# QuEraComputing/tsim

Measured on AMD Instinct MI355X. Metric: detector shots/sec, 35-qubit distillation circuit, 1/2/4/8 MI355X, higher is better.
Workload: dtype int32

## Files before the change

include/tsim_hip.h:

```cpp
#ifndef TSIM_HIP_H
#define TSIM_HIP_H

#include <stdint.h>

#ifdef __cplusplus
extern "C" {
#endif

#define TSIM_OK 0
#define TSIM_EINVAL (-22)
#define TSIM_ENOMEM (-12)
#define TSIM_EHIP (-5)
#define TSIM_ENOTSUP (-95)
#define TSIM_ESTATE (-1)

#define TSIM_MAX_PARAMS 2048

typedef struct tsim_program tsim_program;

typedef struct tsim_level_desc {
  int32_t num_graphs;
  int32_t n_params;
  int32_t ta, tb, tc, td;
  const uint8_t *a_phases;
// ... 303 lines not shown
int tsim_profile_read_stages(tsim_program *p, double stage_ms[3]);
int tsim_profile_read_steps(tsim_program *p, int64_t *steps, int32_t reset);


int tsim_program_info(const tsim_program *p, int32_t *n_components, int32_t *num_outputs,
                      int64_t *image_bytes, int64_t *total_graphs, int64_t *total_rows);

int tsim_program_stats(const tsim_program *p, int64_t out[8]);

#define TSIM_PATH_COUNT 24
int tsim_program_path_counts(tsim_program *p, int64_t out[TSIM_PATH_COUNT], int32_t reset);

const char *tsim_last_error(void);
const char *tsim_version(void);
const char *tsim_tune_keys(void);

#ifdef __cplusplus
}
#endif
#endif
```

tsim_amd/_lib.py:

```python

from __future__ import annotations

import ctypes as C
import os
from pathlib import Path

import numpy as np

_HERE = Path(__file__).resolve().parent
LIB_PATH = _HERE / "libtsim_hip.so"


class HipBackendError(RuntimeError):
    """The HIP extension is missing, failed to load, or a call into it failed."""


class LevelDesc(C.Structure):

    _fields_ = [
        ("num_graphs", C.c_int32),
        ("n_params", C.c_int32),
        ("ta", C.c_int32),
        ("tb", C.c_int32),
        ("tc", C.c_int32),
# ... 178 lines not shown
    "tsim_program_path_counts": (C.c_int, [_P, C.POINTER(_I64), C.c_int32]),
    "tsim_key_split": (None, [_U32, _U32, C.POINTER(_U32)]),
    "tsim_sample_batch_device_begin_split": (C.c_int, [_P, _I32, _P, _I64, _I32, C.POINTER(_U32), _I64, _P, _P, _P, _U32]),
    "tsim_sample_steps_device": (C.c_int, [_P, _I32, C.POINTER(_P), _I64, _I32, C.POINTER(_U32), _I64, C.POINTER(_P), C.POINTER(_P), _U32]),
    "tsim_sample_steps_noise_device": (C.c_int, [_P, _P, _I32, C.POINTER(_P), _I64, _I32, C.POINTER(_U32), C.POINTER(_U32), _I64, C.POINTER(_P),
                                                 C.POINTER(_P), _U32]),
    "tsim_profile_read_steps": (C.c_int, [_P, C.POINTER(_I64), _I32]),
    "tsim_memcpy_d2h_async": (C.c_int, [_P, _P, _P, _I64, _P]),
    "tsim_memcpy_h2d_async": (C.c_int, [_P, _P, _P, _I64, _P]),
    "tsim_stream_synchronize": (C.c_int, [_P, _P]),
    "tsim_aux_stream": (C.c_int, [_P, _I32, C.POINTER(_P)]),
    "tsim_pipeline_next_slot": (C.c_int, [_P, C.POINTER(_I32)]),
    "tsim_last_error": (C.c_char_p, []),
    "tsim_version": (C.c_char_p, []),
    "tsim_tune_keys": (C.c_char_p, []),
}

_lib = None


def load(build: bool = True) -> C.CDLL:
    global _lib
    if _lib is not None:
        return _lib
    path = Path(os.environ.get("TSIM_AMD_LIB", LIB_PATH))
    if path == LIB_PATH:
        from . import build as _build

        if _build.needs_build():
            if path.exists() and os.environ.get("TSIM_AMD_ALLOW_STALE") == "1":
# ... 59 lines not shown
```

tsim_amd/csrc/tsim_internal.hip.h:

```cpp
#pragma once
#include "tsim_host.hip.h"
#include "tsim_kernels.hip.h"
#include "tsim_kernel4.hip.h"
#ifndef TSIM_HARD_NW
#define TSIM_HARD_NW 8
#endif
#include "tsim_lw.hip.h"

#include <algorithm>
#include <array>
#include <cstdarg>
#include <cstdio>
#include <cstdlib>
#include <cmath>
#include <atomic>
#include <mutex>
#include <chrono>
#include <cstring>
#include <functional>
#include <new>
#include <string>
#include <thread>
#include <unordered_set>
#include <vector>

#define TSIMK_H_MAX_CTX 8
constexpr int kListRows = 40;
constexpr int kMinLists = 4;
constexpr int kHardLdsKb = 128;
constexpr int kV4Block = 256;
constexpr int kWideGlobGraphs = 48;

void tsim_parallel_for_impl(size_t n, int max_threads, const std::function<void(size_t)> &fn);
template <class F>
inline void tsim_parallel_for(size_t n, int max_threads, F &&fn) {
  tsim_parallel_for_impl(n, max_threads, std::function<void(size_t)>(std::forward<F>(fn)));
}

namespace tsimhost {

struct FastGraph {
// ... 176 lines not shown
  int lw_direct_left = 0;
  struct Knobs {
    bool adaptive = true;
    bool fused_steps = true;
    int deep_tables = 0;
    bool defer = true;
    int defer_group = 4;
    bool lw_fast = true;
    bool wide_fused = true;
    bool hard_wave = true;
    int hard_wave_rows = 1024;
    long long hard_inline_rows = 1ll << 40;
    bool hard_comp_par = true;
    unsigned long long deep_after = 0;
    int fused_lanes = 0;
    int fused_max = 8;
    bool wide_tables = true;
    bool hard_overflow = true;
    bool shallow = true;
    bool noise_fused = true;
    int trie = 1;
    int gen = 1;
    int x4 = 32;
    bool x3 = true;
    int wide_depth = 4;
    int wide_passes = 8;
    bool wide_compact = true;
  } knobs;
  bool h_attr_set = false;
  bool hm_attr_set = false;
  unsigned gen_attr_set = 0;
// ... 101 lines not shown
```

tsim_amd/csrc/tsim_kernel4.hip.h:

```cpp
#pragma once
#include "tsim_kernels.hip.h"

namespace tsimk {

enum { L4_G = 0, L4_NTILES, L4_TABLES, L4_RECS, L4_NCH, L4_FLAGS, L4_FRAME, L4_STAB, L4_WORDS = 8 };
enum {
  G4_M0 = 0, G4_M1, G4_M3, G4_PM, G4_N1, G4_DBITS , G4_TBL, G4_FLAGS, G4_TBL2,
  G4_CFIELD = 9 ,
  G4_APRE = 11, G4_APIM = 12, G4_WORDS = 16
};
#define TSIMK_G4FLAG_D_COMBINED 1u
#define TSIMK_G4FLAG_D_SEPARATE 2u
enum { C4_LEVELS = 8, C4_WORDS = 16 };

#ifndef TSIMK_V4_WAVES
#define TSIMK_V4_WAVES 1
#endif

struct Sample4Args {
  SampleArgs s;
  int comp4_off;
  int has_check;
  uint32_t *feedback;
};
// ... 335 lines not shown
    }
    if (check_block && threadIdx.x == 0 && active && A.norm_dev) A.norm_dev[ci] = maxdev;
  }

  if (active && !check_block) {
    if (A.out) {
      uint64_t *orow = A.out + row * A.WO;
      for (int w = 0; w < A.WO; ++w)
        orow[w] = (uint64_t)lds_o[(2 * w) * nthr] | ((uint64_t)lds_o[(2 * w + 1) * nthr] << 32);
    }
    store_compact_row(A, row, lds_o, nthr);
  }
}

#ifndef TSIMK_H_MAX_CTX
#define TSIMK_H_MAX_CTX 8
#endif
struct Over4Multi {
  int n_ctx, comp4_off;
  uint32_t slot_begin;
  int masked;
  SampleArgs ctx[TSIMK_H_MAX_CTX];
};

template <int GT, int NCH>
__device__ __forceinline__ void over4_rows(const SampleArgs *ctx, int n_ctx, int comp4_off, uint32_t slot_begin, bool masked,
                                           uint32_t worker, uint32_t n_workers) {
  const uint32_t nthr = blockDim.x;
  __shared__ uint32_t s_cnt[TSIMK_H_MAX_CTX * 64];
  {
    bool any = false;
// ... 41 lines not shown
```

tsim_amd/csrc/tsim_kernel4h.hip.h:

```cpp
#pragma once
#include "tsim_kernel4.hip.h"

namespace tsimk {

#define TSIMK_H_MAX_GROUP_TILES 12

template <int GT, int NCH, int NW>
struct Hard4 {
  static constexpr int kMaxPerWave = (TSIMK_H_MAX_GROUP_TILES * GT + NW - 1) / NW;
  static constexpr int kTileBytes = NCH * Tile4<GT>::kChunkBytes;
  static constexpr int kExchWords = NW * 8 * 64;
};

__device__ __forceinline__ void h4_index(cptr gr, uint32_t U, uint32_t V, uint32_t O1, uint32_t O2, uint32_t &idx,
                                         uint32_t &dbits, uint32_t &r) {
  const uint32_t gflags = gr[G4_FLAGS];
  const bool z = (O1 & gr[G4_M0]) != 0;
  const uint32_t m1 = (uint32_t)__builtin_popcount(O1 & gr[G4_M1]);
  const uint32_t m3 = (uint32_t)__builtin_popcount(O1 & gr[G4_M3]);
  idx = m3 - m1 + gr[G4_N1];
  const uint32_t dsh = gr[G4_DBITS];
  dbits = O2 & ((1u << dsh) - 1u);
  if (gflags & TSIMK_G4FLAG_D_COMBINED) idx = (idx << dsh) | dbits;
  idx = z ? 0u : idx + 1u;
// ... 285 lines not shown
    }
    store_compact_row(A, row, lds_o, 64);
  }
  if (check_block || loop_stride <= 0 || !A.row_index) return;
  __syncthreads();
  }
}

template <int GT, int NCH, int NW>
__global__ void __launch_bounds__(NW * 64) __attribute__((amdgpu_waves_per_eu(3, 8))) k_sample4h(Sample4Args A4, int group_tiles, int loop_stride,
                                                        uint32_t *feedback) {
  sample4h_rows<GT, NCH, NW>(A4.s, A4.comp4_off, A4.has_check != 0, group_tiles, loop_stride, feedback, blockIdx.x,
                             gridDim.x);
}

#define TSIMK_H_MAX_CTX 8
struct Hard4Multi {
  int n_ctx, blocks_per_ctx, group_tiles, loop_stride;
  int comp4_off, check_mask;
  uint32_t *feedback;
  uint32_t main_blocks, over_from;
  SampleArgs ctx[TSIMK_H_MAX_CTX];
};

template <int GT, int NCH, int NW>
__global__ void __launch_bounds__(NW * 64) __attribute__((amdgpu_waves_per_eu(3, 8))) k_sample4h_multi(Hard4Multi M) {
  if (blockIdx.x >= M.main_blocks) {
    over4_rows<GT, NCH>(M.ctx, M.n_ctx, M.comp4_off, M.over_from, false, blockIdx.x - M.main_blocks, gridDim.x - M.main_blocks);
    return;
  }
  const uint32_t c = blockIdx.x / (uint32_t)M.blocks_per_ctx;
// ... 10 lines not shown
```

tsim_amd/csrc/tsim_kernel_hw.hip.h:

```cpp
#pragma once
#include "tsim_kernels.hip.h"
#include "tsim_kernel4.hip.h"

namespace tsimk {

#define TSIMK_HW_MAX_CTX 8
struct HwMulti {
  int n_ctx, waves_per_list, max_lists;
  int comp_par;
  int par_words;
  uint32_t slot_cap;
  uint32_t hw_blocks;
  int comp4_off;
  uint32_t *feedback;
  SampleArgs ctx[TSIMK_HW_MAX_CTX];
};

__device__ __forceinline__ int hw_sum_i32(int v) {
#pragma unroll
  for (int o = 32; o > 0; o >>= 1) v += __shfl_xor(v, o, 64);
  return v;
}
__device__ __forceinline__ uint32_t hw_or_u32(uint32_t v) {
#pragma unroll
// ... 419 lines not shown
```

tsim_amd/csrc/tsim_lw_fast.hip.h:

```cpp
#pragma once
#include "tsim_lw_multi.hip.h"

namespace tsimk {

enum { LWF_NRUNS = 0, LWF_FLIP0, LWF_FLIP1, LWF_RUNS ,
       LWF_RANK , LWF_LUT , LWF_NOUT, LWF_WORDS = 16 };
#define TSIMK_LWF_MAX_RUNS 32
#define TSIMK_LWF_MAX_NOUT 8

__device__ __forceinline__ uint32_t threefry_bits32_lo(uint32_t k0, uint32_t k1, uint32_t k0hi, uint32_t lo) {
  const uint32_t k2 = k0 ^ k1 ^ 0x1BD11BDAu;
  uint32_t x0, x1, t;
#define TF_RN(r) "v_alignbit_b32 %[x1], %[x1], %[x1], " #r "\n v_xor_b32 %[x1], %[x1], %[x0]\n"
#define TF_RA(r) "v_add_u32 %[x0], %[x0], %[x1]\n" TF_RN(r)
#define TF_INJ(kb, i, ka) "s_add_i32 %[t], %[" #kb "], " #i "\n v_add_u32 %[x1], %[t], %[x1]\n v_add3_u32 %[x0], %[x0], %[x1], %[" #ka "]\n"
  asm("v_add_u32 %[x1], %[k1], %[lo]\n v_add_u32 %[x0], %[k0hi], %[x1]\n"
      TF_RN(19) TF_RA(17) TF_RA(6) TF_RA(26)
      TF_INJ(k2, 1, k1) TF_RN(15) TF_RA(3) TF_RA(16) TF_RA(8)
      TF_INJ(k0, 2, k2) TF_RN(19) TF_RA(17) TF_RA(6) TF_RA(26)
      TF_INJ(k1, 3, k0) TF_RN(15) TF_RA(3) TF_RA(16) TF_RA(8)
      TF_INJ(k2, 4, k1) TF_RN(19) TF_RA(17) TF_RA(6) TF_RA(26)
      "s_add_i32 %[t], %[k0], 5\n v_add_u32 %[x0], %[k2], %[x0]\n v_add_u32 %[x1], %[t], %[x1]\n v_xor_b32 %[x0], %[x0], %[x1]\n"
      : [x0] "=&v"(x0), [x1] "=&v"(x1), [t] "=&s"(t)
      : [lo] "v"(lo), [k0] "s"(k0), [k1] "s"(k1), [k2] "s"(k2), [k0hi] "s"(k0hi)
// ... 7 lines not shown
template <int WF32, int NOUT>
__global__ void __launch_bounds__(1024) __attribute__((amdgpu_num_sgpr(TSIMK_LW_SGPRS))) k_sample_lw_fast(LwMultiArgs M) {
  typedef const __attribute__((address_space(4))) uint8_t *cbytes;
  typedef const __attribute__((address_space(4))) LwStep *cstep;
  typedef uint32_t u32x2 __attribute__((ext_vector_type(2)));
  typedef uint32_t u32x4 __attribute__((ext_vector_type(4)));
  constexpr int NPOS = 32 * WF32;
  constexpr int RSTR = NPOS + 1;
  constexpr int L_RANK = 0;
  constexpr int L_LUT = (L_RANK + 8 * RSTR + 1) & ~1;
  constexpr int L_RUNS = L_LUT + (2 << NOUT);
  constexpr int L_BASES = L_RUNS + 4 * TSIMK_LWF_MAX_RUNS;
  constexpr int L_WORDS = L_BASES + 72;
  __shared__ uint32_t lds[L_WORDS];
  const int nthr = blockDim.x;
  cptr img = (cptr)(uintptr_t)M.img;
  cptr rec = img + M.lw_off;
  cptr fr = img + M.lwf_off;
  {
    const uint32_t *g = M.img;
    const uint32_t rank_off = fr[LWF_RANK], lut_off = fr[LWF_LUT], runs_off = fr[LWF_RUNS], n_runs = fr[LWF_NRUNS];
    for (int i = threadIdx.x; i < 8 * RSTR; i += nthr)
      lds[L_RANK + i] = (i % RSTR) < NPOS ? g[rank_off + (uint32_t)(i / RSTR) * 128u + (uint32_t)(i % RSTR)] : 0u;
    for (int i = threadIdx.x; i < (2 << NOUT); i += nthr) lds[L_LUT + i] = g[lut_off + i];
    for (int i = threadIdx.x; i < 4 * TSIMK_LWF_MAX_RUNS; i += nthr) lds[L_RUNS + i] = (uint32_t)i < 4u * n_runs ? g[runs_off + i] : 0u;
    if (threadIdx.x < 72) lds[L_BASES + threadIdx.x] = threadIdx.x < 8 ? g[M.lw_off + LW_BASES_INLINE + threadIdx.x] : 0u;
    __syncthreads();
  }
  const uint32_t n_runs = fr[LWF_NRUNS], flip0 = fr[LWF_FLIP0], flip1 = fr[LWF_FLIP1];
  uint32_t sel[4];
#pragma unroll
  for (int w = 0; w < 4; ++w) sel[w] = w < WF32 ? rec[LW_SEL_INLINE + w] : 0u;
  const uint32_t wmax = rec[LW_WMAX];
  const uint32_t tab_byte = rec[LW_TAB] * 4u;
  const uint32_t keybase = rec[LW_KEYBASE];
  const __amdgpu_buffer_rsrc_t r_tab = __builtin_amdgcn_make_buffer_rsrc((void *)M.tab, 0, M.tab_bytes, 0x00020000);
  cstep steps = (cstep)((cbytes)__builtin_amdgcn_kernarg_segment_ptr() + __builtin_offsetof(LwMultiArgs, step));
  const uint32_t so_lo = (uint32_t)M.shot_offset, so_hi = (uint32_t)((unsigned long long)M.shot_offset >> 32);

  const uint32_t bps = (uint32_t)M.blocks_per_step;
  const uint32_t total = bps * (uint32_t)M.n_steps;
  uint32_t vb = blockIdx.x;
  if (vb >= total) return;
  uint32_t step = vb / bps, rb = vb - step * bps;
  const uint32_t Bu = (uint32_t)M.B;
  uint32_t n[4] = {0u, 0u, 0u, 0u};
  auto load_f = [&](uint32_t st, uint32_t rbk) {
    const __amdgpu_buffer_rsrc_t r_f = __builtin_amdgcn_make_buffer_rsrc((void *)steps[st].f, 0, Bu * (uint32_t)(4 * WF32), 0x00020000);
    const uint32_t row = rbk * (uint32_t)nthr + threadIdx.x;
    const uint32_t off = row * (uint32_t)(4 * WF32);
    if (TSIMK_LWM_SKIP & 64) { n[0] ^= (row * 0x9E3779B9u) & (row * 0x85EBCA6Bu) & (row * 0xC2B2AE35u) & 0x11111111u; n[1] = 0; return; }
    if constexpr (WF32 == 2) {
      const u32x2 v = __builtin_amdgcn_raw_buffer_load_b64(r_f, off, 0, 0);
      n[0] = v.x; n[1] = v.y;
    } else {
      const u32x4 v = __builtin_amdgcn_raw_buffer_load_b128(r_f, off, 0, 0);
      n[0] = v.x; n[1] = v.y; n[2] = v.z; n[3] = v.w;
    }
  };
  load_f(step, rb);
  for (;;) {
    cstep S = steps + step;
    const uint32_t row = rb * (uint32_t)nthr + threadIdx.x;
    const bool active = row < Bu;
    uint32_t f[4] = {n[0], n[1], n[2], n[3]};
    uint32_t vb_n = vb + gridDim.x, step_n = step, rb_n = rb + gridDim.x;
    while (rb_n >= bps) { rb_n -= bps; ++step_n; }
    const bool more = vb_n < total;
    if (more) load_f(step_n, rb_n);
    if (rb == 0u && threadIdx.x <= TSIMK_LW_LISTS)
      S->ctl_next[32u * threadIdx.x] = (threadIdx.x == TSIMK_LW_LISTS) ? 0xFFFFFFFFu : 0u;
    uint32_t o0 = 0u, o1 = 0u;
    for (uint32_t r = 0; r < ((TSIMK_LWM_SKIP & 2) ? 0u : n_runs); ++r) {
      const u32x4 run = *reinterpret_cast<const u32x4 *>(&lds[L_RUNS + 4u * r]);
      const uint32_t sw = (uint32_t)__builtin_amdgcn_readfirstlane((int)run.x) >> 8;
// ... 140 lines not shown
```

tsim_amd/csrc/tsim_lw_multi.hip.h:

```cpp
#pragma once
#include "tsim_lw_pass.hip.h"

namespace tsimk {

#ifndef TSIMK_LWM_SKIP
#define TSIMK_LWM_SKIP 0
#endif

#define TSIMK_LWM_MAX_STEPS 16
#define TSIMK_LWM_KEYS 16

struct LwStep {
  const uint64_t *f;
  uint64_t *out;
  uint8_t *out_compact;
  uint32_t *hard_index;
  uint32_t *ctl;
  uint32_t *ctl_next;
  uint32_t keys[2 * TSIMK_LWM_KEYS];
};

struct LwMultiArgs {
  const uint32_t *img;
  const uint32_t *tab;
  long long B;
  long long shot_offset;
  int n_steps, blocks_per_step;
  int n_comp, lw_off, direct_rot, binom_off;
  int has_check, list_cap, n_lists, out_rb;
  int lwf_off;
  uint32_t tab_bytes;
  int partial;
  LwStep step[TSIMK_LWM_MAX_STEPS];
};

template <int WF32>
__device__ __forceinline__ void lwm_load_f(const uint64_t *f, long long row, bool active, uint32_t &f0, uint32_t &f1, uint32_t &f2,
                                           uint32_t &f3) {
  f0 = f1 = f2 = f3 = 0u;
  if (TSIMK_LWM_SKIP & 64) {
    f0 = ((uint32_t)row * 0x9E3779B9u) & ((uint32_t)row * 0x85EBCA6Bu) & ((uint32_t)row * 0xC2B2AE35u) & 0x11111111u;
    return;
  }
  if (active) {
    const uint64_t *frow = f + row * (WF32 / 2);
    const uint64_t v0 = frow[0];
    f0 = (uint32_t)v0;
// ... 134 lines not shown
```

tsim_amd/csrc/tsim_program.hip:

```cpp
#include "tsim_internal.hip.h"
#include <map>
#include "tsim_sample_internal.hip.h"
#include "tsim_lw_fastm.hip.h"
#include "tsim_kernel4w.hip.h"
#include "tsim_wide.hip.h"
#include "tsim_gen.hip.h"

using namespace tsimk;
using namespace tsimhost;

static thread_local char g_err[512] = "";

bool tsim_debug(const char *what) {
  const char *e = getenv("TSIM_AMD_DEBUG");
  return e && strstr(e, what) != nullptr;
}

int tsim_fail(int code, const char *fmt, ...) {
  va_list ap;
  va_start(ap, fmt);
  vsnprintf(g_err, sizeof g_err, fmt, ap);
  va_end(ap);
  return code;
}
// ... 228 lines not shown
extern "C" int tsim_program_finalize(tsim_program *p, int32_t device) {
  if (!p) return tsim_fail(TSIM_EINVAL, "program is NULL");
  if (p->finalized) return tsim_fail(TSIM_ESTATE, "program already finalized");
  {
    auto env_int = [](const char *name, int dflt) { const char *e = getenv(name); return e ? atoi(e) : dflt; };
    const std::string tune = getenv("TSIM_AMD_TUNE") ? std::string(",") + getenv("TSIM_AMD_TUNE") + "," : std::string();
    auto tune_ll = [&](const char *key, long long dflt) -> long long {
      const std::string k = std::string(",") + key + "=";
      const size_t at = tune.find(k);
      return at == std::string::npos ? dflt : atoll(tune.c_str() + at + k.size());
    };
    p->knobs.adaptive = env_int("TSIM_AMD_ADAPTIVE", 1) != 0;
    p->knobs.fused_steps = env_int("TSIM_AMD_FUSED_STEPS", 1) != 0;
    p->knobs.deep_tables = env_int("TSIM_AMD_DEEP_TABLES", 0);
    p->knobs.defer = tune_ll("defer_hard", 1) != 0;
    p->knobs.defer_group = (int)std::max(0ll, std::min((long long)TSIMK_H_MAX_CTX, tune_ll("defer_group", 0)));
    p->knobs.lw_fast = tune_ll("lw_fast", 1) != 0;
    p->knobs.wide_fused = tune_ll("wide_fused", 1) != 0;
    p->knobs.hard_wave = tune_ll("hard_wave", 1) != 0;
    p->knobs.hard_wave_rows = (int)std::max(0ll, tune_ll("hard_wave_rows", 1024));
    p->knobs.hard_inline_rows = std::max(0ll, tune_ll("hard_inline_rows", 1ll << 40));
    p->knobs.hard_comp_par = tune_ll("hard_comp_par", 1) != 0;
    p->knobs.deep_after = (unsigned long long)std::max(0ll, tune_ll("deep_after", 0));
    p->knobs.fused_lanes = (int)std::max(0ll, std::min(4ll, tune_ll("fused_lanes", 0)));
    p->knobs.fused_max = (int)std::max(1ll, std::min((long long)TSIMK_LWM_MAX_STEPS, tune_ll("fused_max", 8)));
    p->knobs.wide_tables = tune_ll("wide_tables", 1) != 0;
    p->knobs.wide_compact = tune_ll("wide_compact", 1) != 0;
    p->knobs.x3 = tune_ll("x3", 1) != 0;
    p->knobs.x4 = (int)std::max(0ll, tune_ll("x4", 32));
    p->knobs.wide_depth = (int)std::max(0ll, std::min(4ll, tune_ll("wide_depth", 4)));
    p->knobs.wide_passes = (int)std::max(1ll, std::min(16ll, tune_ll("wide_passes", 8)));
    p->knobs.gen = (int)std::max(0ll, std::min(2ll, tune_ll("gen", 1)));
    p->knobs.trie = (int)std::max(0ll, std::min(2ll, tune_ll("trie", 1)));
    p->knobs.noise_fused = tune_ll("noise_fused", 1) != 0;
    p->knobs.shallow = tune_ll("shallow", 1) != 0;
    p->knobs.hard_overflow = tune_ll("hard_overflow", 1) != 0;
  }

  const bool fin_dbg = tsim_debug("finalize");
  auto fin_t0 = std::chrono::steady_clock::now();
// ... 975 lines not shown
        }
      } else {
        p->lw_wmax.clear();
      }
    }
  }
  if (p->lw) {
    while (img.size() % 32) img.push_back(0u);
    p->lw_shadow_off = (int)img.size();
    img.resize(img.size() + p->comps.size() * LW_WORDS, 0u);
  }
  img.resize(img.size() + 256, 0u);
  if (img.size() >= (1ull << 30)) return tsim_fail(TSIM_ENOTSUP, "program image too large");

  if (p->knobs.defer_group <= 0)
    p->knobs.defer_group = p->stats[5] > (4ll << 20) ? TSIMK_H_MAX_CTX : 4;

  fin_mark("pattern-table plan, first-pass records");
  int ndev = 0;
  HIP_TRY(hipGetDeviceCount(&ndev));
  if (device < 0 || device >= ndev) return tsim_fail(TSIM_EINVAL, "device %d out of range (%d visible)", device, ndev);
  p->device = device;
  HIP_TRY(hipSetDevice(device));
  {
    int cu = 0;
    if (hipDeviceGetAttribute(&cu, hipDeviceAttributeMultiprocessorCount, device) == hipSuccess && cu > 0) p->n_cu = cu;
  }
  if (int r = tsim_stream_acquire(device, p->stream_idx, &p->stream)) return r;
  HIP_TRY(hipMalloc((void **)&p->d_img, img.size() * 4));
  HIP_TRY(hipMemcpy(p->d_img, img.data(), img.size() * 4, hipMemcpyHostToDevice));
  HIP_TRY(hipMalloc((void **)&p->d_dev, std::max<size_t>(1, p->comps.size()) * 4));
// ... 285 lines not shown
```

tsim_amd/csrc/tsim_sample.hip:

```cpp
#include "tsim_internal.hip.h"

#include <chrono>
#include "tsim_kernel4h.hip.h"
#include "tsim_filter.hip.h"
#include "tsim_lw_pass.hip.h"
#include "tsim_lw_multi.hip.h"
#include "tsim_lw_fast.hip.h"
#include "tsim_kernel4w.hip.h"
#include "tsim_kernel_hw.hip.h"
#include "tsim_direct.hip.h"
#include "tsim_lw_fastm.hip.h"
#include "tsim_sample_internal.hip.h"
#include "tsim_noise_fused.hip.h"

using namespace tsimk;
using namespace tsimhost;

thread_local TsimNoiseRequest *g_noise_req = nullptr;
HostMarks *g_marks = nullptr;


int prof_event(tsim_program *p, hipStream_t s, int tag) {
  if (p->ev_used == p->ev_pool.size()) {
    hipEvent_t e;
// ... 172 lines not shown
static int slots_now_ready(tsim_program *p) {
  p->slots_ready = true;
  return 0;
}
static thread_local const LaunchPlan *g_carry_plan = nullptr;

void hard_geometry(tsim_program *p, int WF, int WO) {
  constexpr int NW = TSIM_HARD_NW;
  const size_t tile_b = (size_t)p->v4_max_nch * 16 * p->v4_gt * 16;
  const size_t fixed_b = (size_t)(2 * WF + 2 * WO) * 64 * 4 + (size_t)NW * 8 * 64 * 4;
  const size_t budget = (size_t)kHardLdsKb * 1024;
  p->h_group_tiles = fixed_b + tile_b <= budget ? (int)std::min<size_t>(TSIMK_H_MAX_GROUP_TILES, (budget - fixed_b) / tile_b) : 0;
  p->h_lds = fixed_b + (size_t)std::max(1, p->h_group_tiles) * tile_b;
}

static bool hw_eligible(tsim_program *p, const SampleArgs &a, int n_ctx) {
  int wmax = 1;
  for (int w : p->comp_w) wmax = std::max(wmax, w);
  const uint32_t fb_rows = p->h_feedback ? p->h_feedback[0] : 0u;
  return p->fast && p->knobs.hard_wave && wmax <= 4 && a.WF <= 32 && a.WO <= 2 && p->hw_max_rows < 60000 &&
         (unsigned long long)fb_rows * (unsigned)n_ctx <= (unsigned long long)p->knobs.hard_wave_rows;
}
static int launch_over(tsim_program *p, const SampleArgs *ctx, int n_ctx, uint32_t slot_begin, bool masked, hipStream_t hs, bool fill_chip = false) {
  Over4Multi M{};
  M.n_ctx = n_ctx;
  M.comp4_off = p->comp4_off;
  M.slot_begin = slot_begin;
  M.masked = masked ? 1 : 0;
  for (int i = 0; i < n_ctx; ++i) {
    M.ctx[i] = ctx[i];
// ... 1 lines not shown
    M.ctx[i].row_slot_begin = 0;
    M.ctx[i].row_slot_end = 0;
  }
  const int blk = 256;
  const size_t tile_bytes = std::max((size_t)p->v4_max_nch * 16, (size_t)p->v4_max_sent) * p->v4_gt * 16;
  const size_t lds4 = (size_t)(2 * ctx[0].WF + 2 * ctx[0].WO) * blk * 4 + 2 * tile_bytes;
  if (lds4 > (p->v4_max_nch == 32 ? 160 : 64) * 1024) return tsim_fail(TSIM_ENOTSUP, "v4 kernel needs %zu B of LDS", lds4);
  const unsigned grid = (unsigned)p->n_cu * (fill_chip ? (unsigned)std::max<size_t>(1, std::min<size_t>(2048 / blk, (160 * 1024) / (lds4 + 256))) : 1u);
  ++p->path_count[TP_OVER];
  switch (p->v4_max_nch) {
#define TSIM_LO(N) case N: hipLaunchKernelGGL((k_sample4_over<4, N>), dim3(grid), dim3(blk), lds4, hs, M); break;
    TSIM_LO(2) TSIM_LO(4) TSIM_LO(6) TSIM_LO(8) TSIM_LO(10) TSIM_LO(12) TSIM_LO(14) TSIM_LO(20)
#undef TSIM_LO
    case 32: {
      auto kfn = k_sample4_over<4, 32>;
      if (!(p->x4_attr_set & 1u)) { HIP_TRY(hipFuncSetAttribute((const void *)kfn, hipFuncAttributeMaxDynamicSharedMemorySize, 160 * 1024 - 4096)); p->x4_attr_set |= 1u; }
      hipLaunchKernelGGL(kfn, dim3(grid), dim3(blk), lds4, hs, M);
    } break;
    default: hipLaunchKernelGGL((k_sample4_over<4, 16>), dim3(grid), dim3(blk), lds4, hs, M); break;
  }
  HIP_TRY(hipGetLastError());
  return 0;
}
static bool over_available(const tsim_program *p) { return p->v4 && p->knobs.hard_overflow; }

static int launch_hw(tsim_program *p, const SampleArgs *ctx, int n_ctx, int max_lists, hipStream_t hs, bool partial, bool with_feedback = true) {
  int wmax = 1;
  for (int w : p->comp_w) wmax = std::max(wmax, w);
  const uint32_t fb_max = p->h_feedback ? p->h_feedback[1] : 192u;
  HwMulti H{};
  H.n_ctx = n_ctx;
// ... 21 lines not shown
  }
  const int nch = workers ? p->v4_max_nch : 0;
  ++p->path_count[TP_HW];
#define TSIM_LHW(WV, N) case N: hipLaunchKernelGGL((k_sample_hw<WV, N>), dim3(grid), dim3(256), ldsw, hs, H); break;
  if (wmax == 1) switch (nch) {
    TSIM_LHW(1, 0) TSIM_LHW(1, 2) TSIM_LHW(1, 4) TSIM_LHW(1, 6) TSIM_LHW(1, 8) TSIM_LHW(1, 10) TSIM_LHW(1, 12) TSIM_LHW(1, 14) TSIM_LHW(1, 16)
    default: return tsim_fail(TSIM_ESTATE, "bad chunk count %d", nch);
  } else if (wmax > 4) {
    if (nch != 0 || wmax > 8) return tsim_fail(TSIM_ESTATE, "block-per-row kernel: %d parameter words, %d chunks", wmax, nch);
    hipLaunchKernelGGL((k_sample_hw<8, 0>), dim3(grid), dim3(256), ldsw, hs, H);
  } else if (wmax > 2) {
    switch (nch) {
      TSIM_LHW(4, 0) TSIM_LHW(4, 20)
      case 32: {
        auto kfn = k_sample_hw<4, 32>;
        if (!(p->x4_attr_set & 2u)) { HIP_TRY(hipFuncSetAttribute((const void *)kfn, hipFuncAttributeMaxDynamicSharedMemorySize, 160 * 1024 - 4096)); p->x4_attr_set |= 2u; }
        hipLaunchKernelGGL(kfn, dim3(grid), dim3(256), ldsw, hs, H);
      } break;
      default: return tsim_fail(TSIM_ESTATE, "hard-row workers need chunk tables (%d chunks)", nch);
    }
  } else switch (nch) {
    TSIM_LHW(2, 0) TSIM_LHW(2, 2) TSIM_LHW(2, 4) TSIM_LHW(2, 6) TSIM_LHW(2, 8) TSIM_LHW(2, 10) TSIM_LHW(2, 12) TSIM_LHW(2, 14) TSIM_LHW(2, 16)
    default: return tsim_fail(TSIM_ESTATE, "bad chunk count %d", nch);
  }
#undef TSIM_LHW
  HIP_TRY(hipGetLastError());
  return 0;
}

int flush_batch(tsim_program *p) {
  if (p->deferred.empty()) {
// ... 56 lines not shown
  if (cap4h && !over_apart) {
    const size_t tile_bytes = std::max((size_t)p->v4_max_nch * 16, (size_t)p->v4_max_sent) * p->v4_gt * 16;
    lds_m = std::max(lds_m, (size_t)(2 * M.ctx[0].WF + 2 * M.ctx[0].WO) * (NW * 64) * 4 + 2 * tile_bytes);
    grid += (unsigned)p->n_cu * (many ? 2u : 1u);
  }
  if (over_apart) {
    for (hipEvent_t &e : p->over_ev)
      if (!e) HIP_TRY(hipEventCreateWithFlags(&e, hipEventDisableTiming));
    HIP_TRY(hipEventRecord(p->over_ev[0], hs));
  }
  switch (p->v4_max_nch) {
#define TSIM_LHM(N)                                                                                          \
  case N: {                                                                                                  \
    auto kfn = k_sample4h_multi<4, N, NW>;                                                                   \
    if (!p->hm_attr_set)                             \
      HIP_TRY(hipFuncSetAttribute((const void *)kfn, hipFuncAttributeMaxDynamicSharedMemorySize, 156 * 1024)); \
    ++p->path_count[TP_SAMPLE4H_MULTI];                                                                      \
    hipLaunchKernelGGL(kfn, dim3(grid), dim3(NW * 64), lds_m, hs, M);                                        \
  } break;
    TSIM_LHM(2) TSIM_LHM(4) TSIM_LHM(6) TSIM_LHM(8) TSIM_LHM(10) TSIM_LHM(12) TSIM_LHM(14) TSIM_LHM(16) TSIM_LHM(20) TSIM_LHM(32)
#undef TSIM_LHM
    default: return tsim_fail(TSIM_ESTATE, "bad chunk count %d", p->v4_max_nch);
  }
  HIP_TRY(hipGetLastError());
  p->hm_attr_set = true;
  if (over_apart) {
    hipStream_t os = p->slots[4].side != hs ? p->slots[4].side : p->slots[3].side;
    HIP_TRY(hipStreamWaitEvent(os, p->over_ev[0], 0));
    if (int r = launch_over(p, M.ctx, M.n_ctx, cap4h, false, os, true)) return r;
    HIP_TRY(hipEventRecord(p->over_ev[1], os));
    HIP_TRY(hipStreamWaitEvent(hs, p->over_ev[1], 0));
// ... 295 lines not shown
      M.tab = p->d_lw_tab;
      M.B = B;
      M.shot_offset = shot_offset;
      M.n_steps = 1;
      M.blocks_per_step = (int)blocks;
      M.n_comp = (int)p->comps.size();
      M.lw_off = p->lw_off;
      M.direct_rot = p->lw_direct_rot;
      M.binom_off = p->lw_binom_off;
      M.has_check = has_check ? 1 : 0;
      M.list_cap = (int)cap1;
      M.n_lists = n_lists;
      M.out_rb = (p->num_outputs + 7) / 8;
      M.lwf_off = p->lwf_off;
      M.tab_bytes = (uint32_t)p->lw_bytes;
      LwStep &st = M.step[0];
      st.f = a.f;
      st.out = a.out;
      st.out_compact = a.out_compact;
      st.hard_index = l.hard_index;
      st.ctl = l.ctl;
      st.ctl_next = l.ctl_next;
      memcpy(st.keys, a.inline_keys, sizeof(uint32_t) * 2 * (size_t)p->total_keys);
      const long long chip = (long long)p->n_cu * (2048 / blk1);
      const long long it1 = (blocks + chip - 1) / chip;
      const long long gridf = (blocks + it1 - 1) / it1;
      const int n_out = p->comps[0].n_out;
#define TSIM_LF1(N)                                                                                        \
  case N:                                                                                                  \
    if (a.WF == 1) hipLaunchKernelGGL((k_sample_lw_fast<2, N>), dim3((unsigned)gridf), dim3(blk1), 0, s, M); \
// ... 206 lines not shown
        HIP_TRY(hipStreamWaitEvent(s, ev, 0));
      }
    }
  }
  ++p->stat_begins;
  if (plan.defer) ++p->stat_deferred;
  if (!(flags & TSIM_PIPE_INPUTS_READY) && s_user != s) {
    HIP_TRY(hipEventRecord(sl.ev1, s_user));
    HIP_TRY(hipStreamWaitEvent(s, sl.ev1, 0));
  }
  return launch_sample(p, d_f, B, num_f, key_hi, key_lo, shot_offset, d_out, d_max_norm_dev, s, nullptr, nullptr,
                       1 + slot, &plan, (flags & TSIM_PIPE_OUT_BIT_PACKED) != 0);
}


static int steps_group_fused(tsim_program *p, int n, const uint64_t *const *d_f, int64_t B, int32_t num_f, uint32_t key[2],
                             int64_t shot_offset, void *const *d_out, float *const *d_dev, uint32_t flags, const LaunchPlan &plan) {
  const bool packed = (flags & TSIM_PIPE_OUT_BIT_PACKED) != 0;
  if (!p->deferred.empty())
    if (int r = flush_batch(p)) return r;
  const int lanes = p->knobs.fused_lanes > 0 ? p->knobs.fused_lanes : ((long long)n * B <= (1ll << 21) ? 3 : 2);
  hipStream_t s = p->slots[1 + (int)(p->steps_groups++ % (unsigned long long)lanes)].side;
  if (!(flags & TSIM_PIPE_INPUTS_READY) && p->stream != s) {
    if (!p->sync_ev) HIP_TRY(hipEventCreateWithFlags(&p->sync_ev, hipEventDisableTiming));
    HIP_TRY(hipEventRecord(p->sync_ev, p->stream));
    HIP_TRY(hipStreamWaitEvent(s, p->sync_ev, 0));
  }
  const int WF = std::max(1, (num_f + 63) / 64);
  const int blk1 = 1024;
  const long long bps = (B + blk1 - 1) / blk1;
// ... 64 lines not shown
    a.row_slot_end = 0;
  }
  const long long total = bps * n;
  const long long chip = (long long)p->n_cu * (2048 / blk1);
  const long long iters = (total + chip - 1) / chip;
  const long long grid = (total + iters - 1) / iters;
  TSIM_MARK("args");
  if (int r = tsim_tables_slice(p, s)) return r;
  const bool prof = p->profiling && (p->prof_counter++ % p->prof_every == 0);
  if (prof) { if (int r = prof_event(p, s, PROF_BEGIN)) return r; }
  bool part = false;
  const bool fast = p->lwf_off != 0 && p->knobs.lw_fast && B < (1ll << 28) && p->lw_bytes < (1ll << 32) && (n_lists & (n_lists - 1)) == 0 &&
                    ((unsigned long long)shot_offset >> 32) == ((unsigned long long)(shot_offset + B - 1) >> 32);
  M.lwf_off = fast ? p->lwf_off : 0;
  M.tab_bytes = fast ? (uint32_t)p->lw_bytes : 0u;
  TsimNoiseRequest *nq = g_noise_req;
  const bool fuse_noise = nq && fast && nq->fusable && nq->N.WF == WF && (nq->N.tile % blk1) == 0 && p->knobs.noise_fused;
  if (nq && !fuse_noise)
    for (int j = 0; j < n; ++j)
      if (int r = nq->launch(nq->noise, B, nq->keys[2 * (nq->base + j)], nq->keys[2 * (nq->base + j) + 1], const_cast<uint64_t *>(d_f[j]), s)) return r;
  if (fuse_noise) {
    NoiseFusedArgs FA{};
    FA.M = M;
    FA.N = nq->N;
    for (int j = 0; j < n; ++j) {
      FA.nkeys[2 * j] = nq->keys[2 * (nq->base + j)];
      FA.nkeys[2 * j + 1] = nq->keys[2 * (nq->base + j) + 1];
    }
    const long long tiles = ((B + nq->N.tile - 1) / nq->N.tile) * n;
    const long long gridn = std::max<long long>(1, std::min<long long>((long long)p->n_cu * 2, tiles));
// ... 183 lines not shown
          if (int r = slot_prepare(p, k, 0)) return r;
        if (int r = slots_now_ready(p)) return r;
      }
      const int left = n_steps - done;
      const int groups = (left + TSIMK_DIRECT_MAX_STEPS - 1) / TSIMK_DIRECT_MAX_STEPS;
      const int n = (left + groups - 1) / groups;
      if (int r = noise_first(n)) return r;
      if (int r = steps_group_direct(p, n, d_f + done, B, num_f, key, d_out + done, flags)) return r;
      done += n;
      continue;
    }
    LaunchPlan wide_plan;
    bool have_wide_plan = false;
    if (p->knobs.fused_steps && wide_applies(p, B, num_f, shot_offset) && p->series_left == 0) {
      const int left = n_steps - done;
      const int gmax = std::min(TSIMK_LWM_MAX_STEPS, p->knobs.fused_max);
      const int groups = (left + gmax - 1) / gmax;
      const int n = (left + groups - 1) / groups;
      bool okb = true;
      if (flags & TSIM_PIPE_OUT_BIT_PACKED) {
        okb = true;
      } else {
        for (int j = 0; j < n; ++j) okb = okb && !p->slots[1 + (int)((p->steps_slot + (unsigned long long)j) % (unsigned long long)TSIM_PIPELINE_SLOTS)].compact_out;
      }
      if (okb) {
        if (!p->slots_ready) {
          for (int k = 1; k <= 4; ++k)
            if (int r = slot_prepare(p, k, 0)) return r;
          if (int r = slots_now_ready(p)) return r;
        }
        const LaunchPlan wplan = make_plan(p, false, true, (unsigned long long)n * (unsigned long long)B);
// ... 9 lines not shown
        have_wide_plan = true;
      }
    }
    LaunchPlan plan;
    bool have_plan = false;
    if (have_wide_plan) {
      plan = wide_plan;
      have_plan = true;
    }
    if (fused) {
      if (!p->slots_ready) {
        for (int k = 1; k <= 4; ++k)
          if (int r = slot_prepare(p, k, 0)) return r;
        if (int r = slots_now_ready(p)) return r;
      }
      plan = make_plan(p, false, true, (unsigned long long)std::min(n_steps - done, std::min(TSIMK_LWM_MAX_STEPS, p->knobs.fused_max)) * (unsigned long long)B);
      hard_geometry(p, WF, WO);
      TSIM_MARK("plan");
      have_plan = true;
      fused = (plan.defer || p->narrow_big || p->lw_trie) && plan.use_tables && p->h_group_tiles >= 1;
    }
    if (fused) {
      const int left = n_steps - done;
      const int gmax = std::min(gen_fused ? std::min(TSIMK_GEN_MAX_STEPS, std::max(1, TSIMK_GEN_KEYS / std::max(1, p->total_keys))) : TSIMK_LWM_MAX_STEPS, p->knobs.fused_max);
      const int groups = (left + gmax - 1) / gmax;
      const int n = (left + groups - 1) / groups;
      {
        const size_t hard_bytes = (size_t)(((B + 255) / 256 + TSIMK_LW_LISTS - 1) / TSIMK_LW_LISTS * 1024) * TSIMK_LW_LISTS * 4;
        for (int j = 0; j < n; ++j)
          if (int r = slot_prepare(p, 1 + (int)((p->steps_slot + (unsigned long long)j) % TSIM_PIPELINE_SLOTS), hard_bytes)) return r;
      }
      if (gen_fused) {
        if (int r = noise_first(n)) return r;
        if (int r = steps_group_gen(p, n, d_f + done, B, num_f, key, shot_offset, d_out + done, d_max_norm_dev ? d_max_norm_dev + done : nullptr,
                                    flags, plan))
          return r;
      } else if (int r = steps_group_fused(p, n, d_f + done, B, num_f, key, shot_offset, d_out + done,
                                           d_max_norm_dev ? d_max_norm_dev + done : nullptr, flags, plan))
        return r;
      done += n;
    } else {
// ... 305 lines not shown
```

Measured before the change: 77.98 billion.

## Fuse up to 16 steps for long runs and pass lw-fast header via kernargs

Raises the default fused-step cap and max context count to 16, adding a helper that picks 16-step groups only when many steps remain and the group covers enough shots, otherwise keeping the old balanced grouping of at most 8. The lw-fast kernel header fields (offsets, flips, selectors, table base) are read on the host and passed as kernel arguments instead of being loaded from the program image in the kernel. The LDS table preload is moved after the first frame load and rewritten as one strided load per thread, which overlaps with that load. Slightly lowers dynamic LDS limits to fit the larger context structs. This trades larger kernarg structs and possible LDS pressure for fewer launches and less prologue latency.

```diff
diff --git a/include/tsim_hip.h b/include/tsim_hip.h
--- a/include/tsim_hip.h
+++ b/include/tsim_hip.h
@@ -341,6 +341,7 @@
 const char *tsim_last_error(void);
 const char *tsim_version(void);
 const char *tsim_tune_keys(void);
+int32_t tsim_steps_next_group(int32_t left, int64_t B, int32_t fused_max, int64_t long_shots);
 
 #ifdef __cplusplus
 }
diff --git a/tsim_amd/_lib.py b/tsim_amd/_lib.py
--- a/tsim_amd/_lib.py
+++ b/tsim_amd/_lib.py
@@ -216,6 +216,7 @@
     "tsim_last_error": (C.c_char_p, []),
     "tsim_version": (C.c_char_p, []),
     "tsim_tune_keys": (C.c_char_p, []),
+    "tsim_steps_next_group": (_I32, [_I32, _I64, _I32, _I64]),
 }
 
 _lib = None
diff --git a/tsim_amd/csrc/tsim_internal.hip.h b/tsim_amd/csrc/tsim_internal.hip.h
--- a/tsim_amd/csrc/tsim_internal.hip.h
+++ b/tsim_amd/csrc/tsim_internal.hip.h
@@ -24,7 +24,7 @@
 #include <unordered_set>
 #include <vector>
 
-#define TSIMK_H_MAX_CTX 8
+#define TSIMK_H_MAX_CTX 16
 constexpr int kListRows = 40;
 constexpr int kMinLists = 4;
 constexpr int kHardLdsKb = 128;
@@ -231,7 +231,8 @@
     bool hard_comp_par = true;
     unsigned long long deep_after = 0;
     int fused_lanes = 0;
-    int fused_max = 8;
+    int fused_max = 16;
+    long long fused_long_shots = 1ll << 23;
     bool wide_tables = true;
     bool hard_overflow = true;
     bool shallow = true;
diff --git a/tsim_amd/csrc/tsim_kernel4.hip.h b/tsim_amd/csrc/tsim_kernel4.hip.h
--- a/tsim_amd/csrc/tsim_kernel4.hip.h
+++ b/tsim_amd/csrc/tsim_kernel4.hip.h
@@ -373,7 +373,7 @@
 }
 
 #ifndef TSIMK_H_MAX_CTX
-#define TSIMK_H_MAX_CTX 8
+#define TSIMK_H_MAX_CTX 16
 #endif
 struct Over4Multi {
   int n_ctx, comp4_off;
diff --git a/tsim_amd/csrc/tsim_kernel4h.hip.h b/tsim_amd/csrc/tsim_kernel4h.hip.h
--- a/tsim_amd/csrc/tsim_kernel4h.hip.h
+++ b/tsim_amd/csrc/tsim_kernel4h.hip.h
@@ -323,7 +323,7 @@
                              gridDim.x);
 }
 
-#define TSIMK_H_MAX_CTX 8
+#define TSIMK_H_MAX_CTX 16
 struct Hard4Multi {
   int n_ctx, blocks_per_ctx, group_tiles, loop_stride;
   int comp4_off, check_mask;
diff --git a/tsim_amd/csrc/tsim_kernel_hw.hip.h b/tsim_amd/csrc/tsim_kernel_hw.hip.h
--- a/tsim_amd/csrc/tsim_kernel_hw.hip.h
+++ b/tsim_amd/csrc/tsim_kernel_hw.hip.h
@@ -4,7 +4,7 @@
 
 namespace tsimk {
 
-#define TSIMK_HW_MAX_CTX 8
+#define TSIMK_HW_MAX_CTX 16
 struct HwMulti {
   int n_ctx, waves_per_list, max_lists;
   int comp_par;
diff --git a/tsim_amd/csrc/tsim_lw_fast.hip.h b/tsim_amd/csrc/tsim_lw_fast.hip.h
--- a/tsim_amd/csrc/tsim_lw_fast.hip.h
+++ b/tsim_amd/csrc/tsim_lw_fast.hip.h
@@ -45,26 +45,13 @@
   constexpr int L_WORDS = L_BASES + 72;
   __shared__ uint32_t lds[L_WORDS];
   const int nthr = blockDim.x;
-  cptr img = (cptr)(uintptr_t)M.img;
-  cptr rec = img + M.lw_off;
-  cptr fr = img + M.lwf_off;
-  {
-    const uint32_t *g = M.img;
-    const uint32_t rank_off = fr[LWF_RANK], lut_off = fr[LWF_LUT], runs_off = fr[LWF_RUNS], n_runs = fr[LWF_NRUNS];
-    for (int i = threadIdx.x; i < 8 * RSTR; i += nthr)
-      lds[L_RANK + i] = (i % RSTR) < NPOS ? g[rank_off + (uint32_t)(i / RSTR) * 128u + (uint32_t)(i % RSTR)] : 0u;
-    for (int i = threadIdx.x; i < (2 << NOUT); i += nthr) lds[L_LUT + i] = g[lut_off + i];
-    for (int i = threadIdx.x; i < 4 * TSIMK_LWF_MAX_RUNS; i += nthr) lds[L_RUNS + i] = (uint32_t)i < 4u * n_runs ? g[runs_off + i] : 0u;
-    if (threadIdx.x < 72) lds[L_BASES + threadIdx.x] = threadIdx.x < 8 ? g[M.lw_off + LW_BASES_INLINE + threadIdx.x] : 0u;
-    __syncthreads();
-  }
-  const uint32_t n_runs = fr[LWF_NRUNS], flip0 = fr[LWF_FLIP0], flip1 = fr[LWF_FLIP1];
+  const uint32_t n_runs = M.fh.n_runs, flip0 = M.fh.flip0, flip1 = M.fh.flip1;
   uint32_t sel[4];
 #pragma unroll
-  for (int w = 0; w < 4; ++w) sel[w] = w < WF32 ? rec[LW_SEL_INLINE + w] : 0u;
-  const uint32_t wmax = rec[LW_WMAX];
-  const uint32_t tab_byte = rec[LW_TAB] * 4u;
-  const uint32_t keybase = rec[LW_KEYBASE];
+  for (int w = 0; w < 4; ++w) sel[w] = w < WF32 ? M.fh.sel[w] : 0u;
+  const uint32_t wmax = M.fh.wmax;
+  const uint32_t tab_byte = M.fh.tab_byte;
+  const uint32_t keybase = M.fh.keybase;
   const __amdgpu_buffer_rsrc_t r_tab = __builtin_amdgcn_make_buffer_rsrc((void *)M.tab, 0, M.tab_bytes, 0x00020000);
   cstep steps = (cstep)((cbytes)__builtin_amdgcn_kernarg_segment_ptr() + __builtin_offsetof(LwMultiArgs, step));
   const uint32_t so_lo = (uint32_t)M.shot_offset, so_hi = (uint32_t)((unsigned long long)M.shot_offset >> 32);
@@ -90,6 +77,23 @@
     }
   };
   load_f(step, rb);
+  {
+    const uint32_t *g = M.img;
+    const uint32_t t = threadIdx.x;
+    const bool in_rank = t < 8u * (uint32_t)NPOS, in_lut = t < (2u << NOUT), in_runs = t < 4u * n_runs, in_bases = t < 8u;
+    const uint32_t rk = t / (uint32_t)NPOS, rp = t % (uint32_t)NPOS;
+    uint32_t v_rank = 0u, v_lut = 0u, v_runs = 0u, v_bases = 0u;
+    if (in_rank) v_rank = g[M.fh.rank_off + rk * 128u + rp];
+    if (in_lut) v_lut = g[M.fh.lut_off + t];
+    if (in_runs) v_runs = g[M.fh.runs_off + t];
+    if (in_bases) v_bases = g[M.lw_off + LW_BASES_INLINE + t];
+    if (in_rank) lds[L_RANK + rk * (uint32_t)RSTR + rp] = v_rank;
+    if (t < 8u) lds[L_RANK + t * (uint32_t)RSTR + (uint32_t)NPOS] = 0u;
+    if (in_lut) lds[L_LUT + t] = v_lut;
+    if (t < 4u * TSIMK_LWF_MAX_RUNS) lds[L_RUNS + t] = v_runs;
+    if (t < 72u) lds[L_BASES + t] = v_bases;
+    __syncthreads();
+  }
   for (;;) {
     cstep S = steps + step;
     const uint32_t row = rb * (uint32_t)nthr + threadIdx.x;
diff --git a/tsim_amd/csrc/tsim_lw_multi.hip.h b/tsim_amd/csrc/tsim_lw_multi.hip.h
--- a/tsim_amd/csrc/tsim_lw_multi.hip.h
+++ b/tsim_amd/csrc/tsim_lw_multi.hip.h
@@ -20,6 +20,13 @@
   uint32_t keys[2 * TSIMK_LWM_KEYS];
 };
 
+struct LwFastHeader {
+  uint32_t rank_off, lut_off, runs_off, n_runs;
+  uint32_t flip0, flip1;
+  uint32_t wmax, tab_byte, keybase;
+  uint32_t sel[4];
+};
+
 struct LwMultiArgs {
   const uint32_t *img;
   const uint32_t *tab;
@@ -31,6 +38,7 @@
   int lwf_off;
   uint32_t tab_bytes;
   int partial;
+  LwFastHeader fh;
   LwStep step[TSIMK_LWM_MAX_STEPS];
 };
 
diff --git a/tsim_amd/csrc/tsim_program.hip b/tsim_amd/csrc/tsim_program.hip
--- a/tsim_amd/csrc/tsim_program.hip
+++ b/tsim_amd/csrc/tsim_program.hip
@@ -266,7 +266,7 @@
     p->knobs.fused_steps = env_int("TSIM_AMD_FUSED_STEPS", 1) != 0;
     p->knobs.deep_tables = env_int("TSIM_AMD_DEEP_TABLES", 0);
     p->knobs.defer = tune_ll("defer_hard", 1) != 0;
-    p->knobs.defer_group = (int)std::max(0ll, std::min((long long)TSIMK_H_MAX_CTX, tune_ll("defer_group", 0)));
+    p->knobs.defer_group = (int)std::max(0ll, std::min(8ll, tune_ll("defer_group", 0)));
     p->knobs.lw_fast = tune_ll("lw_fast", 1) != 0;
     p->knobs.wide_fused = tune_ll("wide_fused", 1) != 0;
     p->knobs.hard_wave = tune_ll("hard_wave", 1) != 0;
@@ -275,7 +275,12 @@
     p->knobs.hard_comp_par = tune_ll("hard_comp_par", 1) != 0;
     p->knobs.deep_after = (unsigned long long)std::max(0ll, tune_ll("deep_after", 0));
     p->knobs.fused_lanes = (int)std::max(0ll, std::min(4ll, tune_ll("fused_lanes", 0)));
-    p->knobs.fused_max = (int)std::max(1ll, std::min((long long)TSIMK_LWM_MAX_STEPS, tune_ll("fused_max", 8)));
+    p->knobs.fused_max = (int)std::max(1ll, std::min((long long)TSIMK_LWM_MAX_STEPS, tune_ll("fused_max", TSIMK_LWM_MAX_STEPS)));
+    {
+      const size_t at = tune.find(",fused_max=");
+      const size_t colon = at == std::string::npos ? at : tune.find_first_of(":,", at + 1);
+      if (colon != std::string::npos && tune[colon] == ':') p->knobs.fused_long_shots = std::max(0ll, atoll(tune.c_str() + colon + 1));
+    }
     p->knobs.wide_tables = tune_ll("wide_tables", 1) != 0;
     p->knobs.wide_compact = tune_ll("wide_compact", 1) != 0;
     p->knobs.x3 = tune_ll("x3", 1) != 0;
@@ -1281,7 +1286,7 @@
   if (img.size() >= (1ull << 30)) return tsim_fail(TSIM_ENOTSUP, "program image too large");
 
   if (p->knobs.defer_group <= 0)
-    p->knobs.defer_group = p->stats[5] > (4ll << 20) ? TSIMK_H_MAX_CTX : 4;
+    p->knobs.defer_group = p->stats[5] > (4ll << 20) ? 8 : 4;
 
   fin_mark("pattern-table plan, first-pass records");
   int ndev = 0;
diff --git a/tsim_amd/csrc/tsim_sample.hip b/tsim_amd/csrc/tsim_sample.hip
--- a/tsim_amd/csrc/tsim_sample.hip
+++ b/tsim_amd/csrc/tsim_sample.hip
@@ -210,6 +210,21 @@
   p->h_lds = fixed_b + (size_t)std::max(1, p->h_group_tiles) * tile_b;
 }
 
+static void lwf_fill_header(const tsim_program *p, LwMultiArgs &M) {
+  const uint32_t *fr = &p->img[(size_t)p->lwf_off], *rec = &p->img[(size_t)p->lw_off];
+  LwFastHeader &h = M.fh;
+  h.rank_off = fr[LWF_RANK];
+  h.lut_off = fr[LWF_LUT];
+  h.runs_off = fr[LWF_RUNS];
+  h.n_runs = fr[LWF_NRUNS];
+  h.flip0 = fr[LWF_FLIP0];
+  h.flip1 = fr[LWF_FLIP1];
+  h.wmax = rec[LW_WMAX];
+  h.tab_byte = rec[LW_TAB] * 4u;
+  h.keybase = rec[LW_KEYBASE];
+  for (int w = 0; w < 4; ++w) h.sel[w] = rec[LW_SEL_INLINE + w];
+}
+
 static bool hw_eligible(tsim_program *p, const SampleArgs &a, int n_ctx) {
   int wmax = 1;
   for (int w : p->comp_w) wmax = std::max(wmax, w);
@@ -241,7 +256,7 @@
 #undef TSIM_LO
     case 32: {
       auto kfn = k_sample4_over<4, 32>;
-      if (!(p->x4_attr_set & 1u)) { HIP_TRY(hipFuncSetAttribute((const void *)kfn, hipFuncAttributeMaxDynamicSharedMemorySize, 160 * 1024 - 4096)); p->x4_attr_set |= 1u; }
+      if (!(p->x4_attr_set & 1u)) { HIP_TRY(hipFuncSetAttribute((const void *)kfn, hipFuncAttributeMaxDynamicSharedMemorySize, 160 * 1024 - 8192)); p->x4_attr_set |= 1u; }
       hipLaunchKernelGGL(kfn, dim3(grid), dim3(blk), lds4, hs, M);
     } break;
     default: hipLaunchKernelGGL((k_sample4_over<4, 16>), dim3(grid), dim3(blk), lds4, hs, M); break;
@@ -293,7 +308,7 @@
       TSIM_LHW(4, 0) TSIM_LHW(4, 20)
       case 32: {
         auto kfn = k_sample_hw<4, 32>;
-        if (!(p->x4_attr_set & 2u)) { HIP_TRY(hipFuncSetAttribute((const void *)kfn, hipFuncAttributeMaxDynamicSharedMemorySize, 160 * 1024 - 4096)); p->x4_attr_set |= 2u; }
+        if (!(p->x4_attr_set & 2u)) { HIP_TRY(hipFuncSetAttribute((const void *)kfn, hipFuncAttributeMaxDynamicSharedMemorySize, 160 * 1024 - 8192)); p->x4_attr_set |= 2u; }
         hipLaunchKernelGGL(kfn, dim3(grid), dim3(256), ldsw, hs, H);
       } break;
       default: return tsim_fail(TSIM_ESTATE, "hard-row workers need chunk tables (%d chunks)", nch);
@@ -380,7 +395,7 @@
   case N: {                                                                                                  \
     auto kfn = k_sample4h_multi<4, N, NW>;                                                                   \
     if (!p->hm_attr_set)                             \
-      HIP_TRY(hipFuncSetAttribute((const void *)kfn, hipFuncAttributeMaxDynamicSharedMemorySize, 156 * 1024)); \
+      HIP_TRY(hipFuncSetAttribute((const void *)kfn, hipFuncAttributeMaxDynamicSharedMemorySize, 152 * 1024)); \
     ++p->path_count[TP_SAMPLE4H_MULTI];                                                                      \
     hipLaunchKernelGGL(kfn, dim3(grid), dim3(NW * 64), lds_m, hs, M);                                        \
   } break;
@@ -706,6 +721,7 @@
       M.out_rb = (p->num_outputs + 7) / 8;
       M.lwf_off = p->lwf_off;
       M.tab_bytes = (uint32_t)p->lw_bytes;
+      lwf_fill_header(p, M);
       LwStep &st = M.step[0];
       st.f = a.f;
       st.out = a.out;
@@ -942,6 +958,15 @@
 }
 
 
+extern "C" int32_t tsim_steps_next_group(int32_t left, int64_t B, int32_t fused_max, int64_t long_shots) {
+  if (left <= 0) return 0;
+  const int cap = std::max(1, std::min(TSIMK_LWM_MAX_STEPS, (int)fused_max));
+  if (cap > 8 && left >= 2 * TSIMK_LWM_MAX_STEPS && (long long)cap * (long long)B >= (long long)long_shots) return cap;
+  const int g = std::min(cap, 8);
+  const int groups = (left + g - 1) / g;
+  return (left + groups - 1) / groups;
+}
+
 static int steps_group_fused(tsim_program *p, int n, const uint64_t *const *d_f, int64_t B, int32_t num_f, uint32_t key[2],
                              int64_t shot_offset, void *const *d_out, float *const *d_dev, uint32_t flags, const LaunchPlan &plan) {
   const bool packed = (flags & TSIM_PIPE_OUT_BIT_PACKED) != 0;
@@ -1036,6 +1061,7 @@
                     ((unsigned long long)shot_offset >> 32) == ((unsigned long long)(shot_offset + B - 1) >> 32);
   M.lwf_off = fast ? p->lwf_off : 0;
   M.tab_bytes = fast ? (uint32_t)p->lw_bytes : 0u;
+  if (fast) lwf_fill_header(p, M);
   TsimNoiseRequest *nq = g_noise_req;
   const bool fuse_noise = nq && fast && nq->fusable && nq->N.WF == WF && (nq->N.tile % blk1) == 0 && p->knobs.noise_fused;
   if (nq && !fuse_noise)
@@ -1249,7 +1275,7 @@
     bool have_wide_plan = false;
     if (p->knobs.fused_steps && wide_applies(p, B, num_f, shot_offset) && p->series_left == 0) {
       const int left = n_steps - done;
-      const int gmax = std::min(TSIMK_LWM_MAX_STEPS, p->knobs.fused_max);
+      const int gmax = std::min(8, p->knobs.fused_max);
       const int groups = (left + gmax - 1) / gmax;
       const int n = (left + groups - 1) / groups;
       bool okb = true;
@@ -1289,7 +1315,8 @@
           if (int r = slot_prepare(p, k, 0)) return r;
         if (int r = slots_now_ready(p)) return r;
       }
-      plan = make_plan(p, false, true, (unsigned long long)std::min(n_steps - done, std::min(TSIMK_LWM_MAX_STEPS, p->knobs.fused_max)) * (unsigned long long)B);
+      const int n_long = (reg_fused && !gen_fused) ? (int)tsim_steps_next_group(n_steps - done, B, p->knobs.fused_max, p->knobs.fused_long_shots) : 0;
+      plan = make_plan(p, false, true, (unsigned long long)std::max(n_long, std::min(n_steps - done, std::min(8, p->knobs.fused_max))) * (unsigned long long)B);
       hard_geometry(p, WF, WO);
       TSIM_MARK("plan");
       have_plan = true;
@@ -1297,9 +1324,9 @@
     }
     if (fused) {
       const int left = n_steps - done;
-      const int gmax = std::min(gen_fused ? std::min(TSIMK_GEN_MAX_STEPS, std::max(1, TSIMK_GEN_KEYS / std::max(1, p->total_keys))) : TSIMK_LWM_MAX_STEPS, p->knobs.fused_max);
+      const int gmax = std::min(gen_fused ? std::min(TSIMK_GEN_MAX_STEPS, std::max(1, TSIMK_GEN_KEYS / std::max(1, p->total_keys))) : 8, p->knobs.fused_max);
       const int groups = (left + gmax - 1) / gmax;
-      const int n = (left + groups - 1) / groups;
+      const int n = gen_fused ? (left + groups - 1) / groups : (int)tsim_steps_next_group(left, B, p->knobs.fused_max, p->knobs.fused_long_shots);
       {
         const size_t hard_bytes = (size_t)(((B + 255) / 256 + TSIMK_LW_LISTS - 1) / TSIMK_LW_LISTS * 1024) * TSIMK_LW_LISTS * 4;
         for (int j = 0; j < n; ++j)
```

Result: faster. 80.44 billion (median of 6 runs) (+3.2%).
